# mfouda/epsilon

Measured on AMD Instinct MI355X. Metric: ADMM iters/sec, dense Lasso 1e4x5e4, higher is better.
Workload: dtype f32

## Files before the change

### epsilon_amd/csrc/kernels_gemm_f16split.hip

```cpp
#include <hip/hip_runtime.h>

#include <cmath>
#include <cstdlib>
#include <cstring>
#include <map>
#include <mutex>
#include <tuple>
#include <vector>

#include "kernels.h"
#include "options.h"

namespace eps {
namespace k {

namespace {

typedef _Float16 half8 __attribute__((ext_vector_type(8)));
typedef float f32x16 __attribute__((ext_vector_type(16)));

constexpr int TS = 256;
constexpr int SK = 32;
constexpr int LROW = 40;
constexpr int kThreads = 512;

__global__ __launch_bounds__(256) void RowAbsMaxKernel(const float* __restrict__ A, int64_t M, int64_t K,
                                                       int64_t lda, unsigned* __restrict__ rowmax_bits) {
  const int64_t i = blockIdx.x * 256ll + threadIdx.x;
  if (i >= M) return;
  const int64_t per = (K + gridDim.y - 1) / gridDim.y;
  const int64_t k0 = blockIdx.y * per;
  int64_t k1 = k0 + per;
  if (k1 > K) k1 = K;
  float mx = 0.0f;
  const float* p = A + i;
  int64_t k = k0;
  for (; k + 4 <= k1; k += 4) {
    const float a = p[k * lda], b = p[(k + 1) * lda], c = p[(k + 2) * lda], d = p[(k + 3) * lda];
    mx = fmaxf(fmaxf(mx, fmaxf(fabsf(a), fabsf(b))), fmaxf(fabsf(c), fabsf(d)));
  }
  for (; k < k1; ++k) mx = fmaxf(mx, fabsf(p[k * lda]));
  atomicMax(rowmax_bits + i, __float_as_uint(mx));
}

__device__ inline float SplitScaleInv(unsigned amax_bits) {
  const float amax = __uint_as_float(amax_bits);
  if (!(amax > 0.0f) || !isfinite(amax)) return 1.0f;
  int e;
  frexpf(amax, &e);
  int se = 11 - e;
  if (se > 120) se = 120;
  return ldexpf(1.0f, -se);
}

__device__ inline float SplitScale(unsigned amax_bits) {
  const float amax = __uint_as_float(amax_bits);
  if (!(amax > 0.0f) || !isfinite(amax)) return 1.0f;
  int e;
  frexpf(amax, &e);
  int se = 11 - e;
  if (se > 120) se = 120;
  return ldexpf(1.0f, se);
}

__global__ __launch_bounds__(256) void SplitConvertKernel(const float* __restrict__ A, int64_t M, int64_t K,
                                                          int64_t lda, int64_t m_pad,
                                                          const unsigned* __restrict__ rowmax_bits,
                                                          _Float16* __restrict__ H, _Float16* __restrict__ L) {
  __shared__ float tile[SK][65];
  const int64_t i0 = static_cast<int64_t>(blockIdx.x) * 64;
  const int64_t ks = blockIdx.y;
  const int t = threadIdx.x;
  {
    const int r = t & 63, kq = t >> 6;
    const float s = i0 + r < M ? SplitScale(rowmax_bits[i0 + r]) : 1.0f;
#pragma unroll
    for (int p = 0; p < SK / 4; ++p) {
      const int kk = kq + 4 * p;
      const int64_t i = i0 + r, k = ks * SK + kk;
      tile[kk][r] = (i < M && k < K) ? A[i + k * lda] * s : 0.0f;
    }
  }
  __syncthreads();
  {
    const int r = t >> 2, seg = t & 3;
    half8 h, l;
#pragma unroll
    for (int j = 0; j < 8; ++j) {
      const float v = tile[seg * 8 + j][r];
      const _Float16 hv = static_cast<_Float16>(v);
      h[j] = hv;
      l[j] = static_cast<_Float16>(v - static_cast<float>(hv));
    }
    const int64_t off = ((ks * m_pad + i0 + r) * SK) + seg * 8;
    if (i0 + r < m_pad) {
      *reinterpret_cast<half8*>(H + off) = h;
      *reinterpret_cast<half8*>(L + off) = l;
    }
  }
}

__global__ __launch_bounds__(256) void RowAbsMaxKKernel(const float* __restrict__ X, int64_t R, int64_t K,
                                                        int64_t ld, unsigned* __restrict__ rowmax_bits) {
  const int64_t r = blockIdx.x * 4ll + (threadIdx.x >> 6);
  if (r >= R) return;
  const int lane = threadIdx.x & 63;
  const float* p = X + r * ld;
  float mx = 0.0f;
  for (int64_t k = lane; k < K; k += 64) mx = fmaxf(mx, fabsf(p[k]));
#pragma unroll
  for (int off = 32; off > 0; off >>= 1) mx = fmaxf(mx, __shfl_down(mx, off, 64));
  if (lane == 0) rowmax_bits[r] = __float_as_uint(mx);
}

__global__ __launch_bounds__(256) void SplitConvertKKernel(const float* __restrict__ X, int64_t R, int64_t K,
                                                           int64_t ld, int64_t r_pad,
                                                           const unsigned* __restrict__ rowmax_bits,
                                                           _Float16* __restrict__ H, _Float16* __restrict__ L) {
  const int64_t r = blockIdx.x * 64ll + (threadIdx.x >> 2);
  const int seg = threadIdx.x & 3;
  const int64_t ks = blockIdx.y;
  if (r >= r_pad) return;
  half8 h, l;
  const float s = r < R ? SplitScale(rowmax_bits[r]) : 1.0f;
#pragma unroll
  for (int j = 0; j < 8; ++j) {
    const int64_t k = ks * SK + seg * 8 + j;
    const float v = (r < R && k < K) ? X[k + r * ld] * s : 0.0f;
    const _Float16 hv = static_cast<_Float16>(v);
    h[j] = hv;
    l[j] = static_cast<_Float16>(v - static_cast<float>(hv));
  }
  const int64_t off = ((ks * r_pad + r) * SK) + seg * 8;
  *reinterpret_cast<half8*>(H + off) = h;
  *reinterpret_cast<half8*>(L + off) = l;
}

struct SplitOperand {
  const _Float16* H;
  const _Float16* L;
  const unsigned* rowmax;
  int64_t rows_pad;
};

template <int V>
__global__ __launch_bounds__(kThreads, 2) void GemmSplitF16Kernel(
    int64_t M, int64_t N, int64_t nslab, SplitOperand oa, SplitOperand ob, float alpha, float beta, float* C,
    int64_t ldc, int tri, int64_t lin0, int64_t slab0, int64_t slab_count, float* __restrict__ P,
    const int* __restrict__ order, int64_t perm_limit) {
  const int64_t lin = lin0 + blockIdx.x;
  int64_t I, J;
  if (order != nullptr) {
    int64_t tpos = lin;
    if (lin < perm_limit) {
      const int64_t xcd = lin & 7, slot = lin >> 3;
      tpos = ((((slot >> 5) << 3) + xcd) << 5) + (slot & 31);
    }
    const int w = order[tpos];
    I = w >> 16;
    J = w & 0xffff;
  } else if (tri == 1 || tri == 2) {
    I = static_cast<int64_t>((sqrt(8.0 * static_cast<double>(lin) + 1.0) - 1.0) * 0.5);
    while ((I + 1) * (I + 2) / 2 <= lin) ++I;
    while (I * (I + 1) / 2 > lin) --I;
    J = lin - I * (I + 1) / 2;
  } else if (tri == 4) {
    const int64_t TI = (M + TS - 1) / TS, TJ = (N + TS - 1) / TS;
    I = TI - 1 - lin / TJ;
    J = lin % TJ;
  } else {
    const int64_t TI = (M + TS - 1) / TS;
    I = lin % TI;
    J = lin / TI;
  }
  const int64_t i0 = I * TS, j0 = J * TS;
  int64_t ks0 = slab0, ks1 = slab0 + slab_count;
  if (tri == 2 && i0 / SK > ks0) ks0 = i0 / SK;
  if (tri == 3 && j0 / SK > ks0) ks0 = j0 / SK;
  if (tri == 4 && (i0 + TS + SK - 1) / SK < ks1) ks1 = (i0 + TS + SK - 1) / SK;
  if (P != nullptr) {
    ks0 = slab0 + static_cast<int64_t>(blockIdx.y) * slab_count;
    ks1 = ks0 + slab_count;
  }
  if (ks1 > nslab) ks1 = nslab;

  const int t = threadIdx.x, lane = t & 63, wave = t >> 6;
  const int wi = wave & 1, wj = wave >> 1;
  const int l31 = lane & 31, lh = lane >> 5;

  f32x16 acc[4][2];
#pragma unroll
  for (int a = 0; a < 4; ++a)
#pragma unroll
    for (int b = 0; b < 2; ++b)
#pragma unroll
      for (int r = 0; r < 16; ++r) acc[a][b][r] = 0.0f;

  if constexpr (V == 3) {
    __shared__ __attribute__((aligned(16))) _Float16 ring[4][4][TS * 16];
    const int wave_u = __builtin_amdgcn_readfirstlane(wave);
    const int arr_w = wave_u & 3, pg = wave_u >> 2;
    int src_off[4];
#pragma unroll
    for (int q = 0; q < 4; ++q) {
      const int slot = (pg * 4 + q) * 64 + lane;
      const int row = slot >> 1, seg = (slot & 1) ^ ((row >> 3) & 1);
      src_off[q] = row * SK + seg * 8;
    }
    const _Float16* arr_base = arr_w == 0   ? oa.H + i0 * SK
                               : arr_w == 1 ? oa.L + i0 * SK
                               : arr_w == 2 ? ob.H + j0 * SK
                                            : ob.L + j0 * SK;
    const int64_t arr_stride = (arr_w < 2 ? oa.rows_pad : ob.rows_pad) * SK;
    const int64_t nsteps = ks1 > ks0 ? 2 * (ks1 - ks0) : 0;
    auto stage_src = [&](int64_t step) {
      const int64_t sc = step < nsteps ? step : nsteps - 1;
      return arr_base + (ks0 + (sc >> 1)) * arr_stride + (sc & 1) * 16;
    };
    auto stage_issue = [&](int64_t step, const _Float16* src) {
      _Float16* dst = &ring[step & 3][arr_w][pg * 4 * 512];
#pragma unroll
      for (int q = 0; q < 4; ++q)
        __builtin_amdgcn_global_load_lds((const __attribute__((address_space(1))) void*)(src + src_off[q]),
                                         (__attribute__((address_space(3))) void*)(dst + q * 512), 16, 0, 0);
    };
    auto stage = [&](int64_t step) { stage_issue(step, stage_src(step)); };
    const int sw = (l31 >> 3) & 1;
    const int fragI = (wi * 128 + l31) * 16 + ((lh ^ sw) << 3);
    const int fragJ = (wj * 64 + l31) * 16 + ((lh ^ sw) << 3);
    auto readf = [&](int64_t step, half8(&ih)[4], half8(&il)[4], half8(&jh)[2], half8(&jl)[2]) {
      const _Float16* B = &ring[step & 3][0][0];
#pragma unroll
      for (int b = 0; b < 2; ++b) {
        jh[b] = *reinterpret_cast<const half8*>(B + 2 * TS * 16 + fragJ + b * 512);
        jl[b] = *reinterpret_cast<const half8*>(B + 3 * TS * 16 + fragJ + b * 512);
      }
#pragma unroll
      for (int a = 0; a < 4; ++a) {
        ih[a] = *reinterpret_cast<const half8*>(B + fragI + a * 512);
        il[a] = *reinterpret_cast<const half8*>(B + TS * 16 + fragI + a * 512);
      }
    };
    auto half_step = [&](int ap, const half8(&ih)[4], const half8(&il)[4], const half8(&jh)[2],
                         const half8(&jl)[2]) {
#pragma unroll
      for (int term = 0; term < 3; ++term)
#pragma unroll
        for (int a = ap; a < ap + 2; ++a)
#pragma unroll
          for (int b = 0; b < 2; ++b)
            acc[a][b] = __builtin_amdgcn_mfma_f32_32x32x16_f16(term == 2 ? jl[b] : jh[b], term == 1 ? il[a] : ih[a],
                                                               acc[a][b], 0, 0, 0);
    };
    if (nsteps > 0) {
      half8 aih[4], ail[4], ajh[2], ajl[2], bih[4], bil[4], bjh[2], bjl[2];
      stage(0);
      stage(1);
      stage(2);
      asm volatile("s_waitcnt vmcnt(8)" ::: "memory");
      __builtin_amdgcn_s_barrier();
      readf(0, aih, ail, ajh, ajl);
      auto body = [&](int64_t st, const half8(&cih)[4], const half8(&cil)[4], const half8(&cjh)[2],
                      const half8(&cjl)[2], half8(&nih)[4], half8(&nil)[4], half8(&njh)[2], half8(&njl)[2]) {
        const _Float16* nsrc = stage_src(st + 3);
        half_step(0, cih, cil, cjh, cjl);
        __builtin_amdgcn_sched_barrier(0);
        asm volatile("s_waitcnt vmcnt(4)" ::: "memory");
        __builtin_amdgcn_s_barrier();
        __builtin_amdgcn_sched_barrier(0);
        stage_issue(st + 3, nsrc);
        readf(st + 1, nih, nil, njh, njl);
        half_step(2, cih, cil, cjh, cjl);
#pragma unroll
        for (int i = 0; i < 4; ++i) {
          __builtin_amdgcn_sched_group_barrier(0x008, 1, 0);
          __builtin_amdgcn_sched_group_barrier(0x010, 1, 0);
        }
#pragma unroll
        for (int i = 0; i < 6; ++i) {
          __builtin_amdgcn_sched_group_barrier(0x008, 1, 0);
          __builtin_amdgcn_sched_group_barrier(0x100, 2, 0);
        }
        __builtin_amdgcn_sched_group_barrier(0x008, 2, 0);
        __builtin_amdgcn_sched_barrier(0);
      };
      for (int64_t st = 0; st < nsteps; st += 2) {
        body(st, aih, ail, ajh, ajl, bih, bil, bjh, bjl);
        body(st + 1, bih, bil, bjh, bjl, aih, ail, ajh, ajl);
      }
      asm volatile("s_waitcnt vmcnt(0)" ::: "memory");
    }
    const bool interior = P == nullptr && i0 + TS <= M && j0 + TS <= N && ldc % 4 == 0 &&
                          reinterpret_cast<uintptr_t>(C) % 16 == 0;
    if (interior) {
      float* stage = reinterpret_cast<float*>(&ring[0][0][0]);
      const int row4 = lane * 4;
      float ui[4];
#pragma unroll
      for (int e = 0; e < 4; ++e) ui[e] = SplitScaleInv(oa.rowmax[i0 + row4 + e]);
      __syncthreads();
#pragma unroll 1
      for (int h = 0; h < 2; ++h) {
        if ((wj >> 1) == h) {
#pragma unroll
          for (int a = 0; a < 4; ++a)
#pragma unroll
            for (int b = 0; b < 2; ++b)
#pragma unroll
              for (int r = 0; r < 16; ++r) {
                const int col = (wj & 1) * 64 + b * 32 + (r & 3) + 8 * (r >> 2) + 4 * lh;
                stage[col * TS + wi * 128 + a * 32 + l31] = acc[a][b][r];
              }
        }
        __syncthreads();
#pragma unroll 1
        for (int qb = 0; qb < 16; qb += 8) {
          float4 old[8];
          if (beta != 0.0f) {
#pragma unroll
            for (int q = 0; q < 8; ++q) {
              const int64_t j = j0 + h * 128 + wave + 8 * (qb + q);
              old[q] = *reinterpret_cast<const float4*>(C + i0 + row4 + j * ldc);
            }
          }
#pragma unroll
          for (int q = 0; q < 8; ++q) {
            const int c = wave + 8 * (qb + q);
            const int64_t j = j0 + h * 128 + c;
            const float uj = SplitScaleInv(ob.rowmax[j]);
            const float4 a4 = *reinterpret_cast<const float4*>(stage + c * TS + row4);
            float4 v;
            v.x = alpha * ((ui[0] * a4.x) * uj);
            v.y = alpha * ((ui[1] * a4.y) * uj);
            v.z = alpha * ((ui[2] * a4.z) * uj);
            v.w = alpha * ((ui[3] * a4.w) * uj);
            if (beta != 0.0f) {
              v.x = v.x + beta * old[q].x;
              v.y = v.y + beta * old[q].y;
              v.z = v.z + beta * old[q].z;
              v.w = v.w + beta * old[q].w;
            }
            *reinterpret_cast<float4*>(C + i0 + row4 + j * ldc) = v;
          }
        }
        __syncthreads();
      }
      return;
    }
  } else if constexpr (V >= 1) {
    __shared__ __attribute__((aligned(16))) _Float16 sm2[2][4][TS * SK];
    const int wave_u = __builtin_amdgcn_readfirstlane(wave);
    int src_off[2];
#pragma unroll
    for (int q = 0; q < 2; ++q) {
      const int slot = (wave_u * 2 + q) * 64 + lane;
      const int row = slot >> 2, seg = (slot & 3) ^ ((row >> 2) & 3);
      src_off[q] = row * SK + seg * 8;
    }
    auto stage = [&](int buf, int64_t ks) {
      const _Float16* base[4] = {oa.H + (ks * oa.rows_pad + i0) * SK, oa.L + (ks * oa.rows_pad + i0) * SK,
                                 ob.H + (ks * ob.rows_pad + j0) * SK, ob.L + (ks * ob.rows_pad + j0) * SK};
#pragma unroll
      for (int arr = 0; arr < 4; ++arr)
#pragma unroll
        for (int q = 0; q < 2; ++q)
          __builtin_amdgcn_global_load_lds(
              (const __attribute__((address_space(1))) void*)(base[arr] + src_off[q]),
              (__attribute__((address_space(3))) void*)(&sm2[buf][arr][(wave_u * 2 + q) * 512]), 16, 0, 0);
    };
    int offI[4], offJ[2], swI[4], swJ[2];
#pragma unroll
    for (int a = 0; a < 4; ++a) {
      const int row = wi * 128 + a * 32 + l31;
      offI[a] = row * SK;
      swI[a] = (row >> 2) & 3;
    }
#pragma unroll
    for (int b = 0; b < 2; ++b) {
      const int row = wj * 64 + b * 32 + l31;
      offJ[b] = row * SK;
      swJ[b] = (row >> 2) & 3;
    }
    int cur = 0;
    if (ks0 < ks1) {
      stage(0, ks0);
      asm volatile("s_waitcnt vmcnt(0)" ::: "memory");
      __builtin_amdgcn_s_barrier();
    }
    {
      for (int64_t ks = ks0; ks < ks1; ++ks) {
        if (ks + 1 < ks1) stage(cur ^ 1, ks + 1);
#pragma unroll
        for (int kk = 0; kk < SK; kk += 16) {
          half8 ih[4], il[4], jh[2], jl[2];
          const int seg = kk / 8 + lh;
#pragma unroll
          for (int a = 0; a < 4; ++a) {
            const int off = offI[a] + ((seg ^ swI[a]) << 3);
            ih[a] = *reinterpret_cast<const half8*>(&sm2[cur][0][off]);
            il[a] = *reinterpret_cast<const half8*>(&sm2[cur][1][off]);
          }
#pragma unroll
          for (int b = 0; b < 2; ++b) {
            const int off = offJ[b] + ((seg ^ swJ[b]) << 3);
            jh[b] = *reinterpret_cast<const half8*>(&sm2[cur][2][off]);
            jl[b] = *reinterpret_cast<const half8*>(&sm2[cur][3][off]);
          }
#pragma unroll
          for (int a = 0; a < 4; ++a)
#pragma unroll
            for (int b = 0; b < 2; ++b) {
              acc[a][b] = __builtin_amdgcn_mfma_f32_32x32x16_f16(jh[b], ih[a], acc[a][b], 0, 0, 0);
              acc[a][b] = __builtin_amdgcn_mfma_f32_32x32x16_f16(jh[b], il[a], acc[a][b], 0, 0, 0);
              acc[a][b] = __builtin_amdgcn_mfma_f32_32x32x16_f16(jl[b], ih[a], acc[a][b], 0, 0, 0);
            }
        }
        __builtin_amdgcn_sched_barrier(0);
        asm volatile("s_waitcnt vmcnt(0)" ::: "memory");
        __builtin_amdgcn_s_barrier();
        cur ^= 1;
      }
    }
  } else {
    __shared__ __attribute__((aligned(16))) _Float16 sm[4][TS * LROW];
    half8 pre[4][2];
    auto gload = [&](int64_t ks) {
      const _Float16* hI = oa.H + (ks * oa.rows_pad + i0) * SK;
      const _Float16* lI = oa.L + (ks * oa.rows_pad + i0) * SK;
      const _Float16* hJ = ob.H + (ks * ob.rows_pad + j0) * SK;
      const _Float16* lJ = ob.L + (ks * ob.rows_pad + j0) * SK;
  #pragma unroll
      for (int p = 0; p < 2; ++p) {
        const int q = t + kThreads * p;
        pre[0][p] = *reinterpret_cast<const half8*>(hI + q * 8);
        pre[1][p] = *reinterpret_cast<const half8*>(lI + q * 8);
        pre[2][p] = *reinterpret_cast<const half8*>(hJ + q * 8);
        pre[3][p] = *reinterpret_cast<const half8*>(lJ + q * 8);
      }
    };
    auto lstore = [&]() {
  #pragma unroll
      for (int p = 0; p < 2; ++p) {
        const int q = t + kThreads * p;
        const int off = (q >> 2) * LROW + (q & 3) * 8;
  #pragma unroll
        for (int arr = 0; arr < 4; ++arr) *reinterpret_cast<half8*>(&sm[arr][off]) = pre[arr][p];
      }
    };
    if (ks0 < ks1) gload(ks0);
    for (int64_t ks = ks0; ks < ks1; ++ks) {
      __syncthreads();
      lstore();
      __syncthreads();
      if (ks + 1 < ks1) gload(ks + 1);
  #pragma unroll
      for (int kk = 0; kk < SK; kk += 16) {
        half8 ih[4], il[4], jh[2], jl[2];
  #pragma unroll
        for (int a = 0; a < 4; ++a) {
          const int off = (wi * 128 + a * 32 + l31) * LROW + kk + 8 * lh;
          ih[a] = *reinterpret_cast<const half8*>(&sm[0][off]);
          il[a] = *reinterpret_cast<const half8*>(&sm[1][off]);
        }
  #pragma unroll
        for (int b = 0; b < 2; ++b) {
          const int off = (wj * 64 + b * 32 + l31) * LROW + kk + 8 * lh;
          jh[b] = *reinterpret_cast<const half8*>(&sm[2][off]);
          jl[b] = *reinterpret_cast<const half8*>(&sm[3][off]);
        }
  #pragma unroll
        for (int a = 0; a < 4; ++a)
  #pragma unroll
          for (int b = 0; b < 2; ++b) {
            acc[a][b] = __builtin_amdgcn_mfma_f32_32x32x16_f16(jh[b], ih[a], acc[a][b], 0, 0, 0);
            acc[a][b] = __builtin_amdgcn_mfma_f32_32x32x16_f16(jh[b], il[a], acc[a][b], 0, 0, 0);
            acc[a][b] = __builtin_amdgcn_mfma_f32_32x32x16_f16(jl[b], ih[a], acc[a][b], 0, 0, 0);
          }
      }
    }

  }

  if (P != nullptr) {
    float* pt = P + (static_cast<int64_t>(blockIdx.x) * gridDim.y + blockIdx.y) * (TS * TS);
#pragma unroll
    for (int a = 0; a < 4; ++a) {
      const int il = wi * 128 + a * 32 + l31;
#pragma unroll
      for (int b = 0; b < 2; ++b)
#pragma unroll
        for (int r = 0; r < 16; ++r)
          pt[il + (wj * 64 + b * 32 + (r & 3) + 8 * (r >> 2) + 4 * lh) * TS] = acc[a][b][r];
    }
    return;
  }
#pragma unroll
  for (int b = 0; b < 2; ++b) {
    float uj[16];
#pragma unroll
    for (int r = 0; r < 16; ++r) {
      const int64_t j = j0 + wj * 64 + b * 32 + (r & 3) + 8 * (r >> 2) + 4 * lh;
      uj[r] = SplitScaleInv(ob.rowmax[j < N ? j : N - 1]);
    }
#pragma unroll
    for (int a = 0; a < 4; ++a) {
      const int64_t i = i0 + wi * 128 + a * 32 + l31;
      const int64_t ic = i < M ? i : M - 1;
      const float ui = SplitScaleInv(oa.rowmax[ic]);
      float old[16];
      if (beta != 0.0f) {
#pragma unroll
        for (int r = 0; r < 16; ++r) {
          const int64_t j = j0 + wj * 64 + b * 32 + (r & 3) + 8 * (r >> 2) + 4 * lh;
          old[r] = C[ic + (j < N ? j : N - 1) * ldc];
        }
      }
#pragma unroll
      for (int r = 0; r < 16; ++r) {
        const int64_t j = j0 + wj * 64 + b * 32 + (r & 3) + 8 * (r >> 2) + 4 * lh;
        if (i >= M || j >= N) continue;
        const float v = alpha * ((ui * acc[a][b][r]) * uj[r]);
        C[i + j * ldc] = (beta == 0.0f) ? v : v + beta * old[r];
      }
    }
  }
}

__global__ __launch_bounds__(256) void SyrkSplitTailFixupKernel(int64_t M, int64_t N, int64_t lin0, int S,
                                                                const float* __restrict__ P,
                                                                const unsigned* __restrict__ rowmax_i,
                                                                const unsigned* __restrict__ rowmax_j,
                                                                float alpha, float beta, float* C, int64_t ldc,
                                                                const int* __restrict__ order, int lower) {
  const int64_t lin = lin0 + blockIdx.x;
  int64_t I, Jt;
  if (order != nullptr) {
    I = order[lin] >> 16;
    Jt = order[lin] & 0xffff;
  } else if (lower) {
    I = static_cast<int64_t>((sqrt(8.0 * static_cast<double>(lin) + 1.0) - 1.0) * 0.5);
    while ((I + 1) * (I + 2) / 2 <= lin) ++I;
    while (I * (I + 1) / 2 > lin) --I;
    Jt = lin - I * (I + 1) / 2;
  } else {
    const int64_t TI = (M + TS - 1) / TS;
    I = lin % TI;
    Jt = lin / TI;
  }
  const int64_t i0 = I * TS, j0 = Jt * TS;
  const float* p0 = P + static_cast<int64_t>(blockIdx.x) * S * (TS * TS);
  const int per = TS * TS / static_cast<int>(gridDim.y);
  const int e_begin = static_cast<int>(blockIdx.y) * per;
  for (int e = e_begin + threadIdx.x; e < e_begin + per; e += 256) {
    const int64_t i = i0 + (e & (TS - 1)), j = j0 + (e >> 8);
    if (i >= M || j >= N) continue;
    float sum = p0[e];
    for (int c = 1; c < S; ++c) sum += p0[static_cast<int64_t>(c) * (TS * TS) + e];
    float* dst = C + i + j * ldc;
    const float v = alpha * ((SplitScaleInv(rowmax_i[i]) * sum) * SplitScaleInv(rowmax_j[j]));
    *dst = (beta == 0.0f) ? v : v + beta * (*dst);
  }
}

}

namespace {

struct ConvertedOperand {
  std::shared_ptr<Buffer> h, l, mx;
  SplitOperand op;
};

int StageVariant() {
  const char* e = opt::Raw(opt::kGemmStage);
  if (e == nullptr) return 3;
  if (std::strcmp(e, "reg") == 0) return 0;
  if (std::strcmp(e, "lds") == 0) return 1;
  return 3;
}
bool PatchOrderEnabled() {
  return !opt::Is0(opt::kGemmOrder);
}

const int* TileOrder(int64_t TI, int64_t TJ, bool lower, int64_t* count) {
  struct Entry {
    std::shared_ptr<Buffer> buf;
    int64_t count;
  };
  static std::mutex mu;
  static auto* cache = new std::map<std::tuple<int64_t, int64_t, bool>, Entry>();
  std::lock_guard<std::mutex> lock(mu);
  const auto key = std::make_tuple(TI, TJ, lower);
  auto it = cache->find(key);
  if (it == cache->end()) {
    EPS_CHECK(TI < 65536 && TJ < 65536);
    std::vector<int> h;
    constexpr int64_t PS = 8;
    for (int64_t pr = 0; pr * PS < TI; ++pr)
      for (int64_t pc = 0; pc * PS < TJ; ++pc) {
        if (lower && pc > pr) continue;
        for (int64_t i = pr * PS; i < std::min(TI, (pr + 1) * PS); ++i)
          for (int64_t j = pc * PS; j < std::min(TJ, (pc + 1) * PS); ++j)
            if (!lower || j <= i) h.push_back(static_cast<int>((i << 16) | j));
      }
    Entry e;
    e.count = static_cast<int64_t>(h.size());
    e.buf = Runtime::Get().Alloc(h.size() * sizeof(int));
    hipStream_t st = Runtime::Get().stream();
    EPS_HIP(hipMemcpyAsync(e.buf->p, h.data(), h.size() * sizeof(int), hipMemcpyHostToDevice, st));
    EPS_HIP(hipStreamSynchronize(st));
    it = cache->emplace(key, std::move(e)).first;
  }
  *count = it->second.count;
  return static_cast<const int*>(it->second.buf->p);
}

void LaunchSplit(dim3 grid, int64_t M, int64_t N, int64_t nslab, const SplitOperand& oa, const SplitOperand& ob,
                 float al, float be, float* C, int64_t ldc, int tri, int64_t lin0, int64_t slab0, int64_t slab_count,
                 float* P, const int* order, int64_t perm_limit) {
  hipStream_t s = Runtime::Get().stream();
  const int v = StageVariant();
  if (v == 3)
    hipLaunchKernelGGL(GemmSplitF16Kernel<3>, grid, dim3(kThreads), 0, s, M, N, nslab, oa, ob, al, be, C, ldc, tri,
                       lin0, slab0, slab_count, P, order, perm_limit);
  else if (v == 1)
    hipLaunchKernelGGL(GemmSplitF16Kernel<1>, grid, dim3(kThreads), 0, s, M, N, nslab, oa, ob, al, be, C, ldc, tri,
                       lin0, slab0, slab_count, P, order, perm_limit);
  else
    hipLaunchKernelGGL(GemmSplitF16Kernel<0>, grid, dim3(kThreads), 0, s, M, N, nslab, oa, ob, al, be, C, ldc, tri,
                       lin0, slab0, slab_count, P, order, perm_limit);
}

ConvertedOperand ConvertOperand(const float* X, int64_t rows, int64_t K, int64_t ld, bool contig_r) {
  Runtime& rt = Runtime::Get();
  hipStream_t s = rt.stream();
  ConvertedOperand c;
  const int64_t r_pad = (rows + TS - 1) / TS * TS;
  const int64_t nslab = (K + SK - 1) / SK;
  c.h = rt.Alloc(static_cast<size_t>(nslab) * r_pad * SK * sizeof(_Float16));
  c.l = rt.Alloc(static_cast<size_t>(nslab) * r_pad * SK * sizeof(_Float16));
  c.mx = rt.Alloc(static_cast<size_t>(rows) * sizeof(unsigned));
  _Float16* H = static_cast<_Float16*>(c.h->p);
  _Float16* L = static_cast<_Float16*>(c.l->p);
  unsigned* amax = static_cast<unsigned*>(c.mx->p);
  if (contig_r) {
    EPS_HIP(hipMemsetAsync(amax, 0, static_cast<size_t>(rows) * sizeof(unsigned), s));
    const unsigned gx = static_cast<unsigned>((rows + 255) / 256);
    const unsigned gy = static_cast<unsigned>(
        std::max<int64_t>(1, std::min<int64_t>(std::min<int64_t>(256, K), 2048 / gx)));
    hipLaunchKernelGGL(RowAbsMaxKernel, dim3(gx, gy), dim3(256), 0, s, X, rows, K, ld, amax);
    hipLaunchKernelGGL(SplitConvertKernel, dim3(static_cast<unsigned>(r_pad / 64), static_cast<unsigned>(nslab)),
                       dim3(256), 0, s, X, rows, K, ld, r_pad, amax, H, L);
  } else {
    hipLaunchKernelGGL(RowAbsMaxKKernel, dim3(static_cast<unsigned>((rows + 3) / 4)), dim3(256), 0, s, X, rows, K,
                       ld, amax);
    hipLaunchKernelGGL(SplitConvertKKernel, dim3(static_cast<unsigned>(r_pad / 64), static_cast<unsigned>(nslab)),
                       dim3(256), 0, s, X, rows, K, ld, r_pad, amax, H, L);
  }
  c.op = SplitOperand{H, L, amax, r_pad};
  return c;
}

bool AutoKernelChoice() {
  const char* e = opt::Raw(opt::kGemm);
  return e == nullptr || e[0] == 0 || std::strcmp(e, "auto") == 0;
}

bool SplitEnabled() {
  static const bool off = opt::Is0(opt::kGramF16Split);
  return !off;
}

}

bool GemmSplitF16(bool transA, bool transB, int64_t M, int64_t N, int64_t K, double alpha, const DVec& A,
                  int64_t lda, const DVec& B, int64_t ldb, double beta, const DVec& C, int64_t ldc,
                  bool lower_only) {
  if (!SplitEnabled() || A.dt != F32 || B.dt != F32 || C.dt != F32) return false;
  if (M < 1024 || N < 1024 || K < 256 || static_cast<double>(M) * N * K < 8.0e9) return false;
  if (lower_only && M != N) return false;
  Runtime& rt = Runtime::Get();
  hipStream_t s = rt.stream();
  ProfScope prof(lower_only ? "syrk_f16split" : "gemm_f16split", M * N, K);
  const int64_t nslab = (K + SK - 1) / SK;
  ConvertedOperand ca = ConvertOperand(A.as<float>(), M, K, lda, !transA);
  const bool same = A.data() == B.data() && lda == ldb && transA != transB && M == N;
  ConvertedOperand cb;
  if (!same) cb = ConvertOperand(B.as<float>(), N, K, ldb, transB);
  const SplitOperand& oa = ca.op;
  const SplitOperand& ob = same ? ca.op : cb.op;
  const float al = static_cast<float>(alpha), be = static_cast<float>(beta);
  const int64_t TI = (M + TS - 1) / TS, TJ = (N + TS - 1) / TS;
  int64_t ocount = 0;
  const int* order = PatchOrderEnabled() ? TileOrder(TI, TJ, lower_only, &ocount) : nullptr;
  const int64_t total = lower_only ? TI * (TI + 1) / 2 : TI * TJ;
  const int tri = lower_only ? 1 : 0;
  EPS_CHECK(order == nullptr || ocount == total);
  const int64_t slots = 256;
  int64_t tail = total % slots;
  int S = 1;
  int64_t per = nslab;
  if (nslab >= 64 && total > slots && tail > 0 && tail <= slots / 2) {
    S = static_cast<int>(std::min<int64_t>(8, slots / tail));
    per = (nslab + S - 1) / S;
    S = static_cast<int>((nslab + per - 1) / per);
  } else {
    tail = 0;
  }
  const int64_t full = total - tail;
  if (full > 0)
    LaunchSplit(dim3(static_cast<unsigned>(full)), M, N, nslab, oa, ob, al, be, C.as<float>(), ldc, tri, 0, 0, nslab,
                nullptr, order, full / 256 * 256);
  if (tail > 0) {
    auto pbuf = rt.Alloc(static_cast<size_t>(tail) * S * TS * TS * sizeof(float));
    float* P = static_cast<float*>(pbuf->p);
    LaunchSplit(dim3(static_cast<unsigned>(tail), static_cast<unsigned>(S)), M, N, nslab, oa, ob, al, be,
                C.as<float>(), ldc, tri, full, 0, per, P, order, 0);
    hipLaunchKernelGGL(SyrkSplitTailFixupKernel, dim3(static_cast<unsigned>(tail), 16), dim3(256), 0, s, M, N, full,
                       S, P, oa.rowmax, ob.rowmax, al, be, C.as<float>(), ldc, order, tri);
  }
  EPS_HIP(hipGetLastError());
  return true;
}

bool GemmSplitF16KRange(int kmode, int64_t M, int64_t N, int64_t K, double alpha, const DVec& A, int64_t lda,
                        const DVec& B, int64_t ldb, const DVec& C, int64_t ldc) {
  if (!SplitEnabled() || !AutoKernelChoice() || A.dt != F32 || B.dt != F32 || C.dt != F32) return false;
  if (M < 1024 || N < 1024 || K < 256 || static_cast<double>(M) * N * K < 8.0e9) return false;
  if (kmode != 3 && kmode != 4) return false;
  Runtime& rt = Runtime::Get();
  hipStream_t s = rt.stream();
  ProfScope prof("gemm_f16split_krange", M * N, K);
  const int64_t nslab = (K + SK - 1) / SK;
  ConvertedOperand ca = ConvertOperand(A.as<float>(), M, K, lda, true);
  ConvertedOperand cb = ConvertOperand(B.as<float>(), N, K, ldb, false);
  const int64_t TI = (M + TS - 1) / TS, TJ = (N + TS - 1) / TS;
  LaunchSplit(dim3(static_cast<unsigned>(TI * TJ)), M, N, nslab, ca.op, cb.op, static_cast<float>(alpha), 0.0f,
              C.as<float>(), ldc, kmode, 0, 0, nslab, nullptr, nullptr, 0);
  EPS_HIP(hipGetLastError());
  return true;
}

bool SyrkSplitF16LowerTriangular(int64_t n, const DVec& X, int64_t ldx, const DVec& C, int64_t ldc) {
  if (!SplitEnabled() || !AutoKernelChoice() || X.dt != F32 || C.dt != F32 || n < 2048) return false;
  Runtime& rt = Runtime::Get();
  hipStream_t s = rt.stream();
  ProfScope prof("syrk_f16split_tri", n * n, n);
  const int64_t nslab = (n + SK - 1) / SK;
  ConvertedOperand cx = ConvertOperand(X.as<float>(), n, n, ldx, false);
  const int64_t T = (n + TS - 1) / TS;
  LaunchSplit(dim3(static_cast<unsigned>(T * (T + 1) / 2)), n, n, nslab, cx.op, cx.op, 1.0f, 0.0f, C.as<float>(), ldc,
              2, 0, 0, nslab, nullptr, nullptr, 0);
  EPS_HIP(hipGetLastError());
  return true;
}

}
}
```

### epsilon_amd/csrc/options.cc

```cpp
#include "options.h"

#include <algorithm>
#include <cstdlib>
#include <cstring>
#include <string>

#include "common.h"

namespace eps {
namespace opt {
namespace {

const struct Option {
  Id id;
  const char *env, *key, *words[5], *unset;
} kOptions[] = {
    {kBatchWide, "EPSILON_HIP_BATCH_WIDE", "batch_wide", {"0", "1"}, "0"},
    {kBatchWideMin, "EPSILON_HIP_BATCH_WIDE_MIN"},
    {kBatchZeroTall, "EPSILON_HIP_BATCH_ZERO_TALL", "batch_zero_tall", {"0", "1"}, "0"},
    {kBenchRandom, "EPSILON_HIP_BENCH_RANDOM"},
    {kDevice, "EPSILON_HIP_DEVICE", "device"},
    {kDistInverse, "EPSILON_HIP_DIST_INVERSE"},
    {kDtype, "EPSILON_HIP_DTYPE"},
    {kForceSharded, "EPSILON_HIP_FORCE_SHARDED"},
    {kFused, "EPSILON_HIP_FUSED", "fused"},
    {kFusedBlock, "EPSILON_HIP_FUSED_BLOCK"},
    {kFusedGrid, "EPSILON_HIP_FUSED_GRID"},
    {kFusedMatrix, "EPSILON_HIP_FUSED_MATRIX", "fused_matrix", {"0", "pass", "wide", "auto"}, "auto"},
    {kFusedResident, "EPSILON_HIP_FUSED_RESIDENT_KB", "fused_resident"},
    {kFusedTall, "EPSILON_HIP_FUSED_TALL", "fused_tall", {"0", "1", "auto"}, "auto"},
    {kFusedWhiten, "EPSILON_HIP_FUSED_WHITEN"},
    {kFusedZero, "EPSILON_HIP_FUSED_ZERO", "fused_zero", {"0", "auto"}, "auto"},
    {kFusedZeroRidge, "EPSILON_HIP_FUSED_ZERO_RIDGE", "fused_zero_ridge", {"0", "1", "auto"}, "auto"},
    {kFusedZeroTall, "EPSILON_HIP_FUSED_ZERO_TALL", "fused_zero_tall", {"0", "1", "auto"}, "auto"},
    {kFusedZeroTallSmooth, "EPSILON_HIP_FUSED_ZERO_TALL_SMOOTH", "fused_zero_tall_smooth", {"0", "1", "auto"}, "auto"},
    {kGemm, "EPSILON_HIP_GEMM", "gemm"},
    {kGemmOrder, "EPSILON_HIP_GEMM_ORDER"},
    {kGemmSmall, "EPSILON_HIP_GEMM_SMALL"},
    {kGemmStage, "EPSILON_HIP_GEMM_STAGE"},
    {kGramF16Split, "EPSILON_HIP_GRAM_F16SPLIT"},
    {kGraph, "EPSILON_HIP_GRAPH"},
    {kHostThreads, "EPSILON_HIP_HOST_THREADS"},
    {kInitTrace, "EPSILON_HIP_INIT_TRACE"},
    {kPeerWindowMemory, "EPSILON_HIP_PEER_WINDOW_MEMORY"},
    {kPinnedUpload, "EPSILON_HIP_PINNED_UPLOAD"},
    {kPipelineChecks, "EPSILON_HIP_PIPELINE_CHECKS"},
    {kPotrfTwoKernels, "EPSILON_HIP_POTRF_TWO_KERNELS"},
    {kRccl, "EPSILON_HIP_RCCL"},
    {kRefine, "EPSILON_HIP_REFINE", "refine"},
    {kSegGrid, "EPSILON_HIP_SEG_GRID"},
    {kShardedApply, "EPSILON_HIP_SHARDED_APPLY"},
    {kSvd, "EPSILON_HIP_SVD"},
    {kSvdConfirm, "EPSILON_HIP_SVD_CONFIRM"},
    {kSvdInner, "EPSILON_HIP_SVD_INNER"},
    {kSvdMfma, "EPSILON_HIP_SVD_MFMA"},
    {kSvdNoV, "EPSILON_HIP_SVD_NO_V"},
    {kSvdNsplit, "EPSILON_HIP_SVD_NSPLIT"},
    {kSvdPartial, "EPSILON_HIP_SVD_PARTIAL"},
    {kSvdPartialBackoff, "EPSILON_HIP_SVD_PARTIAL_BACKOFF"},
    {kSvdPolar, "EPSILON_HIP_SVD_POLAR"},
    {kSvdSmallFast, "EPSILON_HIP_SVD_SMALL_FAST"},
    {kSvdSort, "EPSILON_HIP_SVD_SORT"},
    {kSvdTrace, "EPSILON_HIP_SVD_TRACE"},
    {kSvdVerbose, "EPSILON_HIP_SVD_VERBOSE"},
    {kSvdWarm, "EPSILON_HIP_SVD_WARM"},
    {kSymvPacked, "EPSILON_HIP_SYMV_PACKED"},
    {kSyrk2d, "EPSILON_HIP_SYRK_2D"},
    {kSyrkTail, "EPSILON_HIP_SYRK_TAIL"},
};
static_assert(sizeof(kOptions) / sizeof(kOptions[0]) == kNumOptions, "one row per Id");

const Option& Row(Id id) {
  const Option& o = kOptions[id];
  EPS_CHECK(o.id == id);
  return o;
}

int WordIndex(const Option& o, const char* value) {
  std::string list;
  for (int i = 0; o.words[i] != nullptr; ++i) {
    if (std::strcmp(o.words[i], value) == 0) return i;
    if (i > 0) list += o.words[i + 1] != nullptr ? ", " : " or ";
    list += o.words[i];
  }
  EPS_FATAL(o.key << " must be " << list << ", got " << value);
}

int64_t ParseFusedResident(const char* value) {
  if (std::strcmp(value, "auto") == 0) return -1;
  const int64_t cap = int64_t(1) << 40;
  int64_t kb = 0;
  bool ok = value[0] != '\0';
  for (const char* c = value; ok && *c != '\0'; ++c) {
    ok = *c >= '0' && *c <= '9';
    if (ok) kb = std::min(cap, kb * 10 + (*c - '0'));
  }
  if (!ok) EPS_FATAL("fused_resident must be auto or a number of KiB, got " << value);
  return kb * 1024;
}

}

const char* Raw(Id id) { return std::getenv(Row(id).env); }

bool IsSet(Id id) { return Raw(id) != nullptr; }

bool Is0(Id id) {
  const char* e = Raw(id);
  return e != nullptr && e[0] == '0';
}

bool Is1(Id id) {
  const char* e = Raw(id);
  return e != nullptr && e[0] == '1';
}

int Int(Id id, int fallback) {
  const char* e = Raw(id);
  return e != nullptr ? std::atoi(e) : fallback;
}

int Word(Id id) {
  const Option& o = Row(id);
  EPS_CHECK(o.words[0] != nullptr);
  const char* e = std::getenv(o.env);
  return WordIndex(o, e != nullptr ? e : o.unset);
}

void Set(const char* key, const char* value) {
  for (const Option& o : kOptions) {
    if (o.key == nullptr || std::strcmp(o.key, key) != 0) continue;
    if (o.words[0] != nullptr) (void)WordIndex(o, value);
    if (o.id == kFusedResident) (void)ParseFusedResident(value);
    if (o.id == kRefine && std::strcmp(value, "auto") == 0) unsetenv(o.env);
    else setenv(o.env, value, 1);
    return;
  }
  EPS_FATAL("unknown option " << key);
}

int64_t FusedResident() {
  const char* e = Raw(kFusedResident);
  return e == nullptr ? -1 : ParseFusedResident(e);
}

int InitTraceLevel() { return Int(kInitTrace, 0); }

SymvPackedMode SymvPacked() {
  const char* e = Raw(kSymvPacked);
  if (e != nullptr && e[0] == '0') return kSymvPackedOff;
  if (e != nullptr && e[0] == '2') return kSymvPackedFirst;
  return kSymvPackedDefault;
}

int DeviceOrdinal(int fallback) {
  const char* e = Raw(kDevice);
  if (e == nullptr) e = std::getenv("LOCAL_RANK");
  return e != nullptr ? std::atoi(e) : fallback;
}

}
}
```

Before: 3357.

## Add 16x16x32 MFMA ring-staged split-f16 GEMM variant and make it default

Adds a new GEMM kernel variant built on 16x16x32 f16 MFMA instructions in place of 32x32x16, with per-wave tiles of 8x4 fragments. It uses a double-buffered LDS ring filled through global_load_lds, and interleaves LDS reads, global loads and MFMAs with explicit sched_group_barrier hints so that loads overlap with matrix math. The stage option becomes a word list, and auto now picks this variant for every triangle mode. The intent is higher MFMA throughput and better latency hiding in the Gram/GEMM that dominates ADMM setup or iterations. The trade-offs are a larger accumulator register footprint and a hand-tuned schedule that may spill registers or stall.

```diff
diff --git a/epsilon_amd/csrc/kernels_gemm_f16split.hip b/epsilon_amd/csrc/kernels_gemm_f16split.hip
--- a/epsilon_amd/csrc/kernels_gemm_f16split.hip
+++ b/epsilon_amd/csrc/kernels_gemm_f16split.hip
@@ -187,6 +187,206 @@
   const int t = threadIdx.x, lane = t & 63, wave = t >> 6;
   const int wi = wave & 1, wj = wave >> 1;
   const int l31 = lane & 31, lh = lane >> 5;
+
+  if constexpr (V == 4) {
+    typedef float f32x4 __attribute__((ext_vector_type(4)));
+    __shared__ __attribute__((aligned(16))) _Float16 ring32[2][4][TS * SK];
+    const int l15 = lane & 15, kg = lane >> 4;
+    f32x4 acc[8][4];
+#pragma unroll
+    for (int a = 0; a < 8; ++a)
+#pragma unroll
+      for (int b = 0; b < 4; ++b)
+#pragma unroll
+        for (int r = 0; r < 4; ++r) acc[a][b][r] = 0.0f;
+    const int wave_u = __builtin_amdgcn_readfirstlane(wave);
+    const int arr_w = wave_u & 3, pg = wave_u >> 2;
+    const int src_off0 = (pg * 128 + (lane >> 2)) * SK + (((lane & 3) ^ (3 * (lane >> 5))) << 3);
+    const _Float16* arr_base = arr_w == 0   ? oa.H + i0 * SK
+                               : arr_w == 1 ? oa.L + i0 * SK
+                               : arr_w == 2 ? ob.H + j0 * SK
+                                            : ob.L + j0 * SK;
+    const int64_t arr_stride = (arr_w < 2 ? oa.rows_pad : ob.rows_pad) * SK;
+    const int64_t nsteps = ks1 > ks0 ? ks1 - ks0 : 0;
+    auto stage_src = [&](int64_t step) {
+      const int64_t sc = step < nsteps ? step : nsteps - 1;
+      return arr_base + (ks0 + sc) * arr_stride;
+    };
+    auto stage_issue = [&](int64_t step, const _Float16* src) {
+      _Float16* dst = &ring32[step & 1][arr_w][pg * 8 * 512];
+#pragma unroll
+      for (int q = 0; q < 8; ++q)
+        __builtin_amdgcn_global_load_lds(
+            (const __attribute__((address_space(1))) void*)(src + src_off0 + q * 512),
+            (__attribute__((address_space(3))) void*)(dst + q * 512), 16, 0, 0);
+    };
+    const int fpos = (kg ^ (3 * ((l15 >> 3) & 1))) << 3;
+    const int fragI = (wi * 128 + l15) * SK + fpos;
+    const int fragJ = (wj * 64 + l15) * SK + fpos;
+    half8 ih[8], il[8], jh[4], jl[4];
+    auto read_i = [&](int64_t step, int a0) {
+      const _Float16* B = &ring32[step & 1][0][0];
+#pragma unroll
+      for (int a = a0; a < a0 + 4; ++a) {
+        ih[a] = *reinterpret_cast<const half8*>(B + fragI + a * 512);
+        il[a] = *reinterpret_cast<const half8*>(B + TS * SK + fragI + a * 512);
+      }
+    };
+    auto read_j = [&](int64_t step, int b0) {
+      const _Float16* B = &ring32[step & 1][0][0];
+#pragma unroll
+      for (int b = b0; b < b0 + 2; ++b) {
+        jh[b] = *reinterpret_cast<const half8*>(B + 2 * TS * SK + fragJ + b * 512);
+        jl[b] = *reinterpret_cast<const half8*>(B + 3 * TS * SK + fragJ + b * 512);
+      }
+    };
+    auto quarter = [&](int a0, int b0) {
+#pragma unroll
+      for (int term = 0; term < 3; ++term)
+#pragma unroll
+        for (int a = a0; a < a0 + 4; ++a)
+#pragma unroll
+          for (int b = b0; b < b0 + 2; ++b)
+            acc[a][b] = __builtin_amdgcn_mfma_f32_16x16x32_f16(term == 2 ? jl[b] : jh[b], term == 1 ? il[a] : ih[a],
+                                                               acc[a][b], 0, 0, 0);
+    };
+    if (nsteps > 0) {
+      stage_issue(0, stage_src(0));
+      stage_issue(1, stage_src(1));
+      asm volatile("s_waitcnt vmcnt(8)" ::: "memory");
+      __builtin_amdgcn_s_barrier();
+      read_i(0, 0);
+      read_j(0, 0);
+      for (int64_t st = 0; st < nsteps; ++st) {
+        const _Float16* nsrc = stage_src(st + 2);
+        read_j(st, 2);
+        read_i(st, 4);
+        quarter(0, 0);
+        quarter(0, 2);
+#pragma unroll
+        for (int i = 0; i < 12; ++i) {
+          __builtin_amdgcn_sched_group_barrier(0x008, 1, 0);
+          __builtin_amdgcn_sched_group_barrier(0x100, 1, 0);
+        }
+        __builtin_amdgcn_sched_group_barrier(0x008, 36, 0);
+        __builtin_amdgcn_sched_barrier(0);
+        asm volatile("s_waitcnt vmcnt(0) lgkmcnt(0)" ::: "memory");
+        __builtin_amdgcn_s_barrier();
+        __builtin_amdgcn_sched_barrier(0);
+        stage_issue(st + 2, nsrc);
+        read_i(st + 1, 0);
+        quarter(4, 0);
+        read_j(st + 1, 0);
+        quarter(4, 2);
+#pragma unroll
+        for (int i = 0; i < 8; ++i) {
+          __builtin_amdgcn_sched_group_barrier(0x008, 1, 0);
+          __builtin_amdgcn_sched_group_barrier(0x010, 1, 0);
+        }
+#pragma unroll
+        for (int i = 0; i < 8; ++i) {
+          __builtin_amdgcn_sched_group_barrier(0x008, 1, 0);
+          __builtin_amdgcn_sched_group_barrier(0x100, 1, 0);
+        }
+        __builtin_amdgcn_sched_group_barrier(0x008, 8, 0);
+#pragma unroll
+        for (int i = 0; i < 4; ++i) {
+          __builtin_amdgcn_sched_group_barrier(0x100, 1, 0);
+          __builtin_amdgcn_sched_group_barrier(0x008, 1, 0);
+        }
+        __builtin_amdgcn_sched_group_barrier(0x008, 20, 0);
+        __builtin_amdgcn_sched_barrier(0);
+      }
+      asm volatile("s_waitcnt vmcnt(0)" ::: "memory");
+    }
+    const bool interior = P == nullptr && i0 + TS <= M && j0 + TS <= N && ldc % 4 == 0 &&
+                          reinterpret_cast<uintptr_t>(C) % 16 == 0;
+    float* stage = reinterpret_cast<float*>(&ring32[0][0][0]);
+    float* pt = P != nullptr ? P + (static_cast<int64_t>(blockIdx.x) * gridDim.y + blockIdx.y) * (TS * TS) : nullptr;
+    const int row4 = lane * 4;
+    float ui[4];
+#pragma unroll
+    for (int e = 0; e < 4; ++e) {
+      const int64_t i = i0 + (interior ? row4 + e : lane + 64 * e);
+      ui[e] = P != nullptr ? 1.0f : SplitScaleInv(oa.rowmax[i < M ? i : M - 1]);
+    }
+    __syncthreads();
+#pragma unroll 1
+    for (int h = 0; h < 2; ++h) {
+      if ((wj >> 1) == h) {
+#pragma unroll
+        for (int a = 0; a < 8; ++a)
+#pragma unroll
+          for (int b = 0; b < 4; ++b)
+#pragma unroll
+            for (int r = 0; r < 4; ++r)
+              stage[((wj & 1) * 64 + b * 16 + kg * 4 + r) * TS + wi * 128 + a * 16 + l15] = acc[a][b][r];
+      }
+      __syncthreads();
+      if (P != nullptr) {
+#pragma unroll 4
+        for (int q = 0; q < 16; ++q) {
+          const int c = wave + 8 * q;
+          *reinterpret_cast<float4*>(pt + (h * 128 + c) * TS + row4) =
+              *reinterpret_cast<const float4*>(stage + c * TS + row4);
+        }
+      } else if (interior) {
+#pragma unroll 1
+        for (int qb = 0; qb < 16; qb += 8) {
+          float4 old[8];
+          if (beta != 0.0f) {
+#pragma unroll
+            for (int q = 0; q < 8; ++q) {
+              const int64_t j = j0 + h * 128 + wave + 8 * (qb + q);
+              old[q] = *reinterpret_cast<const float4*>(C + i0 + row4 + j * ldc);
+            }
+          }
+#pragma unroll
+          for (int q = 0; q < 8; ++q) {
+            const int c = wave + 8 * (qb + q);
+            const int64_t j = j0 + h * 128 + c;
+            const float uj = SplitScaleInv(ob.rowmax[j]);
+            const float4 a4 = *reinterpret_cast<const float4*>(stage + c * TS + row4);
+            float4 v;
+            v.x = alpha * ((ui[0] * a4.x) * uj);
+            v.y = alpha * ((ui[1] * a4.y) * uj);
+            v.z = alpha * ((ui[2] * a4.z) * uj);
+            v.w = alpha * ((ui[3] * a4.w) * uj);
+            if (beta != 0.0f) {
+              v.x = v.x + beta * old[q].x;
+              v.y = v.y + beta * old[q].y;
+              v.z = v.z + beta * old[q].z;
+              v.w = v.w + beta * old[q].w;
+            }
+            *reinterpret_cast<float4*>(C + i0 + row4 + j * ldc) = v;
+          }
+        }
+      } else {
+#pragma unroll 1
+        for (int q = 0; q < 16; ++q) {
+          const int c = wave + 8 * q;
+          const int64_t j = j0 + h * 128 + c;
+          if (j >= N) break;
+          const float uj = SplitScaleInv(ob.rowmax[j]);
+          float old[4];
+#pragma unroll
+          for (int e = 0; e < 4; ++e) {
+            const int64_t i = i0 + lane + 64 * e;
+            old[e] = (beta != 0.0f && i < M) ? C[i + j * ldc] : 0.0f;
+          }
+#pragma unroll
+          for (int e = 0; e < 4; ++e) {
+            const int64_t i = i0 + lane + 64 * e;
+            if (i >= M) continue;
+            const float v = alpha * ((ui[e] * stage[c * TS + lane + 64 * e]) * uj);
+            C[i + j * ldc] = (beta == 0.0f) ? v : v + beta * old[e];
+          }
+        }
+      }
+      __syncthreads();
+    }
+    return;
+  }
 
   f32x16 acc[4][2];
 #pragma unroll
@@ -347,7 +547,7 @@
       }
       return;
     }
-  } else if constexpr (V >= 1) {
+  } else if constexpr (V == 1) {
     __shared__ __attribute__((aligned(16))) _Float16 sm2[2][4][TS * SK];
     const int wave_u = __builtin_amdgcn_readfirstlane(wave);
     int src_off[2];
@@ -421,7 +621,7 @@
         cur ^= 1;
       }
     }
-  } else {
+  } else if constexpr (V == 0) {
     __shared__ __attribute__((aligned(16))) _Float16 sm[4][TS * LROW];
     half8 pre[4][2];
     auto gload = [&](int64_t ks) {
@@ -571,12 +771,11 @@
   SplitOperand op;
 };
 
-int StageVariant() {
-  const char* e = opt::Raw(opt::kGemmStage);
-  if (e == nullptr) return 3;
-  if (std::strcmp(e, "reg") == 0) return 0;
-  if (std::strcmp(e, "lds") == 0) return 1;
-  return 3;
+int StageVariant(int tri) {
+  static const int kAuto[5] = {4, 4, 4, 4, 4};
+  static const int kWord[5] = {-1, 3, 1, 0, 4};
+  const int v = kWord[opt::Word(opt::kGemmStage)];
+  return v >= 0 ? v : kAuto[tri];
 }
 bool PatchOrderEnabled() {
   return !opt::Is0(opt::kGemmOrder);
@@ -619,8 +818,11 @@
                  float al, float be, float* C, int64_t ldc, int tri, int64_t lin0, int64_t slab0, int64_t slab_count,
                  float* P, const int* order, int64_t perm_limit) {
   hipStream_t s = Runtime::Get().stream();
-  const int v = StageVariant();
-  if (v == 3)
+  const int v = StageVariant(tri);
+  if (v == 4)
+    hipLaunchKernelGGL(GemmSplitF16Kernel<4>, grid, dim3(kThreads), 0, s, M, N, nslab, oa, ob, al, be, C, ldc, tri,
+                       lin0, slab0, slab_count, P, order, perm_limit);
+  else if (v == 3)
     hipLaunchKernelGGL(GemmSplitF16Kernel<3>, grid, dim3(kThreads), 0, s, M, N, nslab, oa, ob, al, be, C, ldc, tri,
                        lin0, slab0, slab_count, P, order, perm_limit);
   else if (v == 1)
diff --git a/epsilon_amd/csrc/options.cc b/epsilon_amd/csrc/options.cc
--- a/epsilon_amd/csrc/options.cc
+++ b/epsilon_amd/csrc/options.cc
@@ -13,7 +13,7 @@
 
 const struct Option {
   Id id;
-  const char *env, *key, *words[5], *unset;
+  const char *env, *key, *words[6], *unset;
 } kOptions[] = {
     {kBatchWide, "EPSILON_HIP_BATCH_WIDE", "batch_wide", {"0", "1"}, "0"},
     {kBatchWideMin, "EPSILON_HIP_BATCH_WIDE_MIN"},
@@ -35,9 +35,9 @@
     {kFusedZeroTall, "EPSILON_HIP_FUSED_ZERO_TALL", "fused_zero_tall", {"0", "1", "auto"}, "auto"},
     {kFusedZeroTallSmooth, "EPSILON_HIP_FUSED_ZERO_TALL_SMOOTH", "fused_zero_tall_smooth", {"0", "1", "auto"}, "auto"},
     {kGemm, "EPSILON_HIP_GEMM", "gemm"},
-    {kGemmOrder, "EPSILON_HIP_GEMM_ORDER"},
+    {kGemmOrder, "EPSILON_HIP_GEMM_ORDER", "gemm_order", {"0", "1"}, "1"},
     {kGemmSmall, "EPSILON_HIP_GEMM_SMALL"},
-    {kGemmStage, "EPSILON_HIP_GEMM_STAGE"},
+    {kGemmStage, "EPSILON_HIP_GEMM_STAGE", "gemm_stage", {"auto", "ring", "lds", "reg", "ring32"}, "auto"},
     {kGramF16Split, "EPSILON_HIP_GRAM_F16SPLIT"},
     {kGraph, "EPSILON_HIP_GRAPH"},
     {kHostThreads, "EPSILON_HIP_HOST_THREADS"},
```

New measurement: 3359 (median of 4 runs). No clear change (+0.0%).
